# chengstone/cchess-zero

Hardware: AMD Instinct MI355X
Metric: MCTS simulations/sec (whole node), playout=1600, 7-block net (higher is better)
Workload: dtype mx6

## Files before the change

### cchess_zero_amd/csrc/cz_conv.hip

```cpp
#include "cz_internal.h"
#include "cz_conv_kernel.h"
#include "cz_trunk_split.h"
#include "cz_trunk_mx.h"
#ifdef CZ_EXPERIMENT_MX2
#include "cz_trunk_mx2.h"
#include <cstdlib>
#endif
#ifdef CZ_EXPERIMENT_MX12
#include "cz_trunk_mx12.h"
#include <cstdlib>
#endif

extern "C" int cz_conv3x3_c128_bf16(cz_ctx *c, const void *in, const void *wpk, const float *bias, const void *residual,
                                    void *out, int B, int relu) {
    using namespace czconv;
    CZ_REQUIRE(c && in && wpk && bias && out && B >= 0, "cz_conv3x3_c128_bf16: null argument");
    if (B == 0) return CZ_OK;
    if (!c->conv_attr_set) {
        CZ_HIP(hipFuncSetAttribute(reinterpret_cast<const void *>(k_conv3x3_c128), hipFuncAttributeMaxDynamicSharedMemorySize, CV_LDS_BYTES));
        c->conv_attr_set = true;
    }
    const int grid = (B + CV_P - 1) / CV_P;
    hipLaunchKernelGGL(k_conv3x3_c128, dim3(grid), dim3(CV_THREADS), CV_LDS_BYTES, c->stream, (const uint16_t *)in,
                       (const uint16_t *)wpk, bias, (const uint16_t *)residual, (uint16_t *)out, B, relu);
    CZ_HIP(hipGetLastError());
    return CZ_OK;
}

static unsigned long long *clock_probe(cz_ctx *c, int grid) {
    if (!c->clock_probe || grid > c->clock_probe_wgs) return nullptr;
    c->clock_probe_last_grid = grid;
    return c->clock_probe;
}

static int launch_tower(cz_ctx *c, const void *in, const void *wpk, const float *bias, void *out, const float *head_w,
                        const float *head_b, float *head_out, int B, int nblocks, const void *planes = nullptr,
                        const void *w0 = nullptr, const float *b0 = nullptr, bool f16 = false) {
    if (head_w && (reinterpret_cast<uintptr_t>(head_w) & 15u)) { cz_set_error("cz_net_trunk: head_w must be 16-byte aligned"); return CZ_EINVAL; }
    using namespace czconv;
    if (B == 0) return CZ_OK;
    if (!c->tower_attr_set) {
        CZ_HIP(hipFuncSetAttribute(reinterpret_cast<const void *>(k_tower8_c128<false, 4>), hipFuncAttributeMaxDynamicSharedMemorySize, T8_LDS_BYTES));
        CZ_HIP(hipFuncSetAttribute(reinterpret_cast<const void *>(k_tower8_c128<true, 4>), hipFuncAttributeMaxDynamicSharedMemorySize, T8_LDS_BYTES));
        c->tower_attr_set = true;
    }
    const int grid = (B + T8_P - 1) / T8_P;
    if (f16)
        hipLaunchKernelGGL((k_tower8_c128<true, 4>), dim3(grid), dim3(T8_THREADS), T8_LDS_BYTES, c->stream, (const uint16_t *)in,
                           (const uint16_t *)wpk, bias, (uint16_t *)out, head_w, head_b, head_out, (const uint16_t *)planes,
                           (const uint16_t *)w0, b0, B, 2 * nblocks, c->batch_count, clock_probe(c, grid));
    else
        hipLaunchKernelGGL((k_tower8_c128<false, 4>), dim3(grid), dim3(T8_THREADS), T8_LDS_BYTES, c->stream, (const uint16_t *)in,
                           (const uint16_t *)wpk, bias, (uint16_t *)out, head_w, head_b, head_out, (const uint16_t *)planes,
                           (const uint16_t *)w0, b0, B, 2 * nblocks, c->batch_count, clock_probe(c, grid));
    CZ_HIP(hipGetLastError());
    return CZ_OK;
}

extern "C" int cz_tower_c128_bf16(cz_ctx *c, const void *in, const void *wpk, const float *bias, void *out, int B, int nblocks) {
    CZ_REQUIRE(c && in && wpk && bias && out && B >= 0 && nblocks >= 1, "cz_tower_c128_bf16: null argument / nblocks < 1");
    return launch_tower(c, in, wpk, bias, out, nullptr, nullptr, nullptr, B, nblocks);
}

extern "C" int cz_tower_heads_c128_bf16(cz_ctx *c, const void *in, const void *wpk, const float *bias, void *trunk_out,
                                        const float *head_w, const float *head_b, float *head_out, int B, int nblocks) {
    CZ_REQUIRE(c && in && wpk && bias && head_w && head_b && head_out && B >= 0 && nblocks >= 1,
               "cz_tower_heads_c128_bf16: null argument / nblocks < 1");
    return launch_tower(c, in, wpk, bias, trunk_out, head_w, head_b, head_out, B, nblocks);
}

extern "C" int cz_net_trunk_bf16(cz_ctx *c, const void *planes16, const void *w0, const float *b0, const void *wpk,
                                 const float *bias, void *trunk_out, const float *head_w, const float *head_b,
                                 float *head_out, int B, int nblocks) {
    CZ_REQUIRE(c && planes16 && w0 && b0 && wpk && bias && B >= 0 && nblocks >= 1 && (trunk_out || head_out),
               "cz_net_trunk_bf16: null argument / nblocks < 1");
    CZ_REQUIRE(!head_out || (head_w && head_b), "cz_net_trunk_bf16: head_out needs head_w and head_b");
    return launch_tower(c, nullptr, wpk, bias, trunk_out, head_w, head_b, head_out, B, nblocks, planes16, w0, b0);
}

extern "C" int cz_net_trunk_f16(cz_ctx *c, const void *planes16, const void *w0, const float *b0, const void *wpk,
                                const float *bias, void *trunk_out, const float *head_w, const float *head_b,
                                float *head_out, int B, int nblocks) {
    CZ_REQUIRE(c && planes16 && w0 && b0 && wpk && bias && B >= 0 && nblocks >= 1 && (trunk_out || head_out),
               "cz_net_trunk_f16: null argument / nblocks < 1");
    CZ_REQUIRE(!head_out || (head_w && head_b), "cz_net_trunk_f16: head_out needs head_w and head_b");
    return launch_tower(c, nullptr, wpk, bias, trunk_out, head_w, head_b, head_out, B, nblocks, planes16, w0, b0, true);
}

extern "C" int cz_net_trunk_split(cz_ctx *c, const void *planes16, const void *w0, const float *b0, const void *wpk,
                                  const float *bias, float *trunk_out, const float *head_w, const float *head_b,
                                  float *head_out, int B, int nblocks, int halves_dtype) {
    using namespace czconv;
    CZ_REQUIRE(c && planes16 && w0 && b0 && wpk && bias && B >= 0 && nblocks >= 1 && (trunk_out || head_out),
               "cz_net_trunk_split: null argument / nblocks < 1");
    CZ_REQUIRE(!head_out || (head_w && head_b), "cz_net_trunk_split: head_out needs head_w and head_b");
    CZ_REQUIRE(halves_dtype == CZ_F16 || halves_dtype == CZ_BF16, "cz_net_trunk_split: halves_dtype must be CZ_F16 or CZ_BF16");
    if (head_w && (reinterpret_cast<uintptr_t>(head_w) & 15u)) { cz_set_error("cz_net_trunk_split: head_w must be 16-byte aligned"); return CZ_EINVAL; }
    if (B == 0) return CZ_OK;
    if (!c->split_attr_set) {
        CZ_HIP(hipFuncSetAttribute(reinterpret_cast<const void *>(k_trunk_split_c128<false>), hipFuncAttributeMaxDynamicSharedMemorySize, XS_LDS_BYTES));
        CZ_HIP(hipFuncSetAttribute(reinterpret_cast<const void *>(k_trunk_split_c128<true>), hipFuncAttributeMaxDynamicSharedMemorySize, XS_LDS_BYTES));
        c->split_attr_set = true;
    }
    const int grid = (B + XS_P - 1) / XS_P;
    if (halves_dtype == CZ_F16)
        hipLaunchKernelGGL((k_trunk_split_c128<true>), dim3(grid), dim3(XS_THREADS), XS_LDS_BYTES, c->stream, (const uint16_t *)wpk, bias,
                           trunk_out, head_w, head_b, head_out, (const uint16_t *)planes16, (const uint16_t *)w0, b0, B, 2 * nblocks,
                           c->batch_count, clock_probe(c, grid));
    else
        hipLaunchKernelGGL((k_trunk_split_c128<false>), dim3(grid), dim3(XS_THREADS), XS_LDS_BYTES, c->stream, (const uint16_t *)wpk, bias,
                           trunk_out, head_w, head_b, head_out, (const uint16_t *)planes16, (const uint16_t *)w0, b0, B, 2 * nblocks,
                           c->batch_count, clock_probe(c, grid));
    CZ_HIP(hipGetLastError());
    return CZ_OK;
}

extern "C" int cz_net_trunk_mx(cz_ctx *c, const void *planes16, const void *w0, const float *b0, const void *wpk, const float *bias,
                               float *trunk_out, const float *head_w, const float *head_b, float *head_out, int B, int nblocks) {
    using namespace czconv;
    CZ_REQUIRE(c && planes16 && w0 && b0 && wpk && bias && B >= 0 && nblocks >= 1 && (trunk_out || head_out),
               "cz_net_trunk_mx: null argument / nblocks < 1");
    CZ_REQUIRE(!head_out || (head_w && head_b), "cz_net_trunk_mx: head_out needs head_w and head_b");
    if (head_w && (reinterpret_cast<uintptr_t>(head_w) & 15u)) { cz_set_error("cz_net_trunk_mx: head_w must be 16-byte aligned"); return CZ_EINVAL; }
    if (reinterpret_cast<uintptr_t>(wpk) & 15u) { cz_set_error("cz_net_trunk_mx: wpk must be 16-byte aligned"); return CZ_EINVAL; }
    if (B == 0) return CZ_OK;
    const int grid = (B + MX_P - 1) / MX_P;
#ifdef CZ_EXPERIMENT_MX12
    {
        const char *e = getenv("CCHESS_MX_KERNEL");
        if (e && e[0] == '1' && e[1] == '2') {
            if (!c->mx2_attr_set) {
                CZ_HIP(hipFuncSetAttribute(reinterpret_cast<const void *>(k_trunk_mx12_c128), hipFuncAttributeMaxDynamicSharedMemorySize, MX_LDS_BYTES));
                c->mx2_attr_set = true;
            }
            hipLaunchKernelGGL(k_trunk_mx12_c128, dim3(grid), dim3(768), MX_LDS_BYTES, c->stream, (const unsigned char *)wpk, bias, trunk_out,
                               head_w, head_b, head_out, (const uint16_t *)planes16, (const uint16_t *)w0, b0, B, 2 * nblocks, c->batch_count,
                               clock_probe(c, grid));
            CZ_HIP(hipGetLastError());
            return CZ_OK;
        }
    }
#endif
#ifdef CZ_EXPERIMENT_MX2
    if (!c->mx_kernel) {
        const char *e = getenv("CCHESS_MX_KERNEL");
        c->mx_kernel = (e && e[0] == '2') ? 2 : 1;
    }
    if (c->mx_kernel == 2) {
        if (!c->mx2_attr_set) {
            CZ_HIP(hipFuncSetAttribute(reinterpret_cast<const void *>(k_trunk_mx2_c128), hipFuncAttributeMaxDynamicSharedMemorySize, MX_LDS_BYTES));
            c->mx2_attr_set = true;
        }
        const size_t need = (size_t)grid * MX2_XBUF_FLOATS_PER_WG * sizeof(float);
        if (need > c->mx_xbuf_bytes) {
            CZ_HIP(hipStreamSynchronize(c->stream));
            if (c->mx_xbuf) (void)hipFree(c->mx_xbuf);
            c->mx_xbuf = nullptr; c->mx_xbuf_bytes = 0;
            if (hipMalloc(&c->mx_xbuf, need) != hipSuccess) { c->mx_xbuf = nullptr; cz_set_error("cz_net_trunk_mx: hipMalloc(%zu B) for the block-input scratch failed", need); return CZ_ENOMEM; }
            c->mx_xbuf_bytes = need;
        }
        hipLaunchKernelGGL(k_trunk_mx2_c128, dim3(grid), dim3(MX_THREADS), MX_LDS_BYTES, c->stream, (const unsigned char *)wpk, bias, trunk_out,
                           head_w, head_b, head_out, (const uint16_t *)planes16, (const uint16_t *)w0, b0, B, 2 * nblocks, c->batch_count,
                           clock_probe(c, grid), (float *)c->mx_xbuf);
        CZ_HIP(hipGetLastError());
        return CZ_OK;
    }
#endif
    if (!c->mx_attr_set) {
        CZ_HIP(hipFuncSetAttribute(reinterpret_cast<const void *>(k_trunk_mx_c128), hipFuncAttributeMaxDynamicSharedMemorySize, MX_LDS_BYTES));
        c->mx_attr_set = true;
    }
    hipLaunchKernelGGL(k_trunk_mx_c128, dim3(grid), dim3(MX_THREADS), MX_LDS_BYTES, c->stream, (const unsigned char *)wpk, bias, trunk_out,
                       head_w, head_b, head_out, (const uint16_t *)planes16, (const uint16_t *)w0, b0, B, 2 * nblocks, c->batch_count,
                       clock_probe(c, grid));
    CZ_HIP(hipGetLastError());
    return CZ_OK;
}

extern "C" int cz_set_clock_probe(cz_ctx *c, unsigned long long *buf_dev, int max_workgroups) {
    CZ_REQUIRE(c && max_workgroups >= 0, "cz_set_clock_probe: null context");
    c->clock_probe = buf_dev;
    c->clock_probe_wgs = buf_dev ? max_workgroups : 0;
    c->clock_probe_last_grid = 0;
    return CZ_OK;
}

extern "C" int cz_clock_probe_last_grid(cz_ctx *c) { return c ? c->clock_probe_last_grid : 0; }
```

### cchess_zero_amd/csrc/cz_internal.h

```cpp
#pragma once
#include <cstddef>
#include <hip/hip_runtime.h>
#include <math.h>
#include <stdint.h>
#include <stdio.h>
#include <string>

#include "../../include/cchess_hip.h"
#include "cz_device.h"

void cz_set_error(const char *fmt, ...);
#define CZ_HIP(expr)                                                                              \
    do {                                                                                          \
        hipError_t _e = (expr);                                                                   \
        if (_e != hipSuccess) {                                                                   \
            cz_set_error("%s failed: %s (%s:%d)", #expr, hipGetErrorString(_e), __FILE__, __LINE__); \
            return CZ_EHIP;                                                                       \
        }                                                                                         \
    } while (0)
#define CZ_REQUIRE(cond, msg)                                \
    do {                                                     \
        if (!(cond)) { cz_set_error("%s", msg); return CZ_EINVAL; } \
    } while (0)

struct CzHostTables {
    char labels[CZ_NLABELS * 5];
    int16_t lut[CZ_NSQ * CZ_NSQ];
    int16_t unflip[CZ_NLABELS];
    uint16_t srcdst[CZ_NLABELS];
    uint64_t zob[15 * CZ_NSQ + 1];
};
const CzHostTables &cz_host_tables();

#define CZ_PATH_MAX 32

struct CzPool {
    float *P, *W, *Q;
    int32_t *N, *parent, *child_begin;
    uint16_t *child_count, *move;
    uint16_t *sd;
};

struct CzSelfplay {
    int max_plies;
    uint8_t *hist;
    int32_t *ply;
    uint8_t *stalled;
    uint8_t *active;
    uint8_t *start_board;
    uint8_t *start_side;
    int32_t *start_rr;
    long long *stats;
};

#define CZ_EC_BUCKETS 128
#define CZ_XC_BUSY (1ull << 63)
#define CZ_EC_ENTRIES (CZ_EC_BUCKETS * 64)
#ifndef CZ_EC_BUDGET
#define CZ_EC_BUDGET 4
#endif

struct CzTreeRec {
    int32_t root_rr, root_node, n_nodes, status;
    int32_t sims;
    int16_t last_depth;
    uint16_t root_ply;
    int32_t pend_kind, pend_leaf;
    float pend_value;
    int32_t pend_depth;
    uint32_t ec_hits, ec_lookups;
    unsigned long long pend_key;
    uint16_t pend_nmoves;
    uint8_t root_side, pend_side;
    uint32_t ec_collisions;
};
static_assert(sizeof(CzTreeRec) == 64, "CzTreeRec is one 64-byte line per tree");

template <typename T, int OFF>
struct CzRecField {
    char *base;
    __host__ __device__ __forceinline__ T &operator[](int g) const { return *reinterpret_cast<T *>(base + (size_t)g * sizeof(CzTreeRec) + OFF); }
};
#define CZ_REC_FIELD(type, name) CzRecField<type, offsetof(CzTreeRec, name)> name

struct CzTrees {
    CzPool pool;
    int cap;
    int words;
    unsigned long long *mark_bits;
    uint32_t *mark_rank;
    int32_t *adv_list, *adv_cnt;
    uint8_t *root_board;
    union {
        CzTreeRec *rec;
        CZ_REC_FIELD(int32_t, root_rr); CZ_REC_FIELD(int32_t, root_node); CZ_REC_FIELD(int32_t, n_nodes);
        CZ_REC_FIELD(int32_t, status); CZ_REC_FIELD(int32_t, sims); CZ_REC_FIELD(int16_t, last_depth); CZ_REC_FIELD(uint16_t, root_ply);
        CZ_REC_FIELD(int32_t, pend_kind); CZ_REC_FIELD(int32_t, pend_leaf); CZ_REC_FIELD(float, pend_value);
        CZ_REC_FIELD(int32_t, pend_depth); CZ_REC_FIELD(uint32_t, ec_hits); CZ_REC_FIELD(uint32_t, ec_lookups); CZ_REC_FIELD(uint32_t, ec_collisions);
        CZ_REC_FIELD(unsigned long long, pend_key); CZ_REC_FIELD(uint16_t, pend_nmoves);
        CZ_REC_FIELD(uint8_t, root_side); CZ_REC_FIELD(uint8_t, pend_side);
    };
    uint16_t *pend_moves;
    int32_t *pend_path;
    int32_t *pk_kind, *pk_leaf;
    float *pk_value;
    uint8_t *pk_side;
    uint16_t *pk_nmoves;
    unsigned long long *ec_key;
    int32_t *ec_node;
    float *ec_val;
    uint32_t *ec_board;
    uint32_t *pend_board;
    unsigned long long ec_key_mask;
    char *xc_base;
    uint32_t xc_mask;
    int32_t *slot_of;
    int32_t *evcnt;
    unsigned long long *evtotal;
};

struct cz_ctx {
    int device;
    hipStream_t stream;
    int max_games, cap, G;
    CzTables tab;
    void *tab_block;
    CzTrees t;
    void *tree_block;
    void *pool_block;
    bool adv_attr_set;
    bool adv_force_global;
    bool conv_attr_set, tower_attr_set, split_attr_set, mx_attr_set;
#if defined(CZ_EXPERIMENT_MX2) || defined(CZ_EXPERIMENT_MX12)
    bool mx2_attr_set;
    int mx_kernel;
    void *mx_xbuf;
    size_t mx_xbuf_bytes;
#endif
    int width;
    void *pend_block;
    int terminal_extra;
    int sim_target;
    int step_parity;
    const int32_t *batch_count;
    void *xc_block;
    int xc_log2_entries;
    const struct CzmTables *mask_tab;
    unsigned long long *clock_probe;
    int clock_probe_wgs, clock_probe_last_grid;
    CzSelfplay sp;
    void *sp_block;
    void *ec_block;
};

__host__ __device__ __forceinline__ size_t czx_n(const CzTrees &t) { return ((size_t)t.xc_mask + 1) * 64; }
__host__ __device__ __forceinline__ unsigned long long *czx_key(const CzTrees &t) { return reinterpret_cast<unsigned long long *>(t.xc_base); }
__host__ __device__ __forceinline__ uint32_t *czx_tree_stats(const CzTrees &t) { return reinterpret_cast<uint32_t *>(t.xc_base + czx_n(t) * 1088 + 64); }
__host__ __device__ __forceinline__ float *czx_val(const CzTrees &t) { return reinterpret_cast<float *>(t.xc_base + czx_n(t) * 8 + 64); }
__host__ __device__ __forceinline__ uint32_t *czx_cnt(const CzTrees &t) { return reinterpret_cast<uint32_t *>(t.xc_base + czx_n(t) * 12 + 64); }
__host__ __device__ __forceinline__ uint32_t *czx_board(const CzTrees &t) { return reinterpret_cast<uint32_t *>(t.xc_base + czx_n(t) * 16 + 64); }
__host__ __device__ __forceinline__ uint16_t *czx_moves(const CzTrees &t) { return reinterpret_cast<uint16_t *>(t.xc_base + czx_n(t) * 64 + 64); }
__host__ __device__ __forceinline__ uint16_t *czx_sd(const CzTrees &t) { return reinterpret_cast<uint16_t *>(t.xc_base + czx_n(t) * 320 + 64); }
__host__ __device__ __forceinline__ float *czx_P(const CzTrees &t) { return reinterpret_cast<float *>(t.xc_base + czx_n(t) * 576 + 64); }

struct TreeView {
    float *P, *W, *Q;
    int32_t *N, *parent, *child_begin;
    uint16_t *child_count, *move;
    uint16_t *sd;
};

__device__ __forceinline__ TreeView view_of(const CzTrees &t, int g) {
    const CzPool &p = t.pool;
    const size_t base = (size_t)g * (size_t)t.cap;
    TreeView v;
    v.P = p.P + base; v.W = p.W + base; v.Q = p.Q + base;
    v.N = p.N + base; v.parent = p.parent + base; v.child_begin = p.child_begin + base;
    v.child_count = p.child_count + base; v.move = p.move + base; v.sd = p.sd + base;
    return v;
}

__device__ __forceinline__ void init_root(TreeView v, int idx) {
    v.P[idx] = 1.0f;
    v.W[idx] = 0.f; v.Q[idx] = 0.f; v.N[idx] = 0; v.parent[idx] = -1; v.child_begin[idx] = -1;
    v.child_count[idx] = 0; v.move[idx] = 0xFFFF; v.sd[idx] = 0;
}

__device__ __forceinline__ void ec_clear_tree(const CzTrees &t, int g, int tid, int nthreads) {
    if (!t.ec_key) return;
    unsigned long long *k = t.ec_key + (size_t)g * CZ_EC_ENTRIES;
    for (int i = tid; i < CZ_EC_ENTRIES; i += nthreads) k[i] = 0ull;
}

__device__ __forceinline__ void fresh_root(const CzTrees &t, int g, int lane) {
    if (lane == 0) {
        t.root_node[g] = 0; t.n_nodes[g] = 1; t.status[g] = 0; t.sims[g] = 0; t.last_depth[g] = 0; t.root_ply[g] = 0;
        t.pend_kind[g] = 0; t.pend_leaf[g] = 0; t.pend_value[g] = 0.f; t.pend_side[g] = 0; t.pend_nmoves[g] = 0;
        init_root(view_of(t, g), 0);
    }
    ec_clear_tree(t, g, lane, 64);
}
__device__ __forceinline__ void fresh_root(const CzTrees &t, int g, int lane, const uint8_t *__restrict__ boards, int stride,
                                           const uint8_t *__restrict__ side, const int32_t *__restrict__ rr, int i) {
    for (int j = lane; j < CZD_BOARD_LDS; j += 64)
        t.root_board[(size_t)g * CZD_BOARD_LDS + j] = j < CZ_NSQ ? boards[(size_t)i * stride + j] : (uint8_t)0;
    if (lane == 0) { t.root_side[g] = side[i] ? 1 : 0; t.root_rr[g] = rr ? rr[i] : 0; }
    fresh_root(t, g, lane);
}

__device__ __forceinline__ void wave_kings_missing(const uint8_t *board, int lane, bool &Kmiss, bool &kmiss) {
    const int c0 = board[lane], c1 = (lane + 64 < CZ_NSQ) ? board[lane + 64] : 0;
    Kmiss = __ballot(c0 == 1 || c1 == 1) == 0ull;
    kmiss = __ballot(c0 == 8 || c1 == 8) == 0ull;
}
__device__ __forceinline__ int king_capture_winner(bool Kmiss) { return Kmiss ? 1 : 0; }
__device__ __forceinline__ bool restrict_round_draw(int rr) { return rr >= 60; }

__device__ __forceinline__ void root_children(const CzTrees &t, int g, const TreeView &v, int &cb, int &n) {
    const int root = t.root_node[g];
    cb = v.child_begin[root];
    n = cb < 0 ? 0 : (int)v.child_count[root];
}
__device__ __forceinline__ bool root_cannot_move(int status, int n) {
    return n == 0 || (status & (CZ_ST_NO_MOVES | CZ_ST_MOVE_OVERFLOW)) != 0;
}

__device__ __forceinline__ int wave_most_visited(const TreeView &v, int cb, int n, int lane) {
    int bn = -1, bi = 0x7fffffff;
    for (int i = lane; i < n; i += 64) {
        const int x = v.N[cb + i];
        if (x > bn) { bn = x; bi = i; }
    }
#pragma unroll
    for (int d = 32; d >= 1; d >>= 1) {
        const int on = __shfl_xor(bn, d, 64), oi = __shfl_xor(bi, d, 64);
        if (on > bn || (on == bn && oi < bi)) { bn = on; bi = oi; }
    }
    return bi;
}

__device__ __forceinline__ double wave_sum(double x) {
#pragma unroll
    for (int d = 32; d >= 1; d >>= 1) x += __shfl_xor(x, d, 64);
    return x;
}
__device__ __forceinline__ double wave_max(double x) {
#pragma unroll
    for (int d = 32; d >= 1; d >>= 1) x = fmax(x, __shfl_xor(x, d, 64));
    return x;
}
__device__ __forceinline__ double wave_incl_scan(double v, int lane) {
    double x = v;
#pragma unroll
    for (int d = 1; d < 64; d <<= 1) {
        const double y = __shfl_up(x, d, 64);
        if (lane >= d) x += y;
    }
    return x;
}

__device__ __forceinline__ void wave_visit_policy(const int N[2], int n, double inv_temp, int lane, double pi[2]) {
    double x[2], e[2];
#pragma unroll
    for (int r = 0; r < 2; ++r) {
        const int i = lane + 64 * r;
        x[r] = (i < n && N[r] > 0) ? inv_temp * log((double)N[r]) : -INFINITY;
    }
    const double m = wave_max(fmax(x[0], x[1]));
#pragma unroll
    for (int r = 0; r < 2; ++r) e[r] = (x[r] == -INFINITY || m == -INFINITY) ? 0.0 : exp(x[r] - m);
    const double se = wave_sum(e[0] + e[1]);
#pragma unroll
    for (int r = 0; r < 2; ++r) {
        const int i = lane + 64 * r;
        pi[r] = se > 0.0 ? e[r] / se : (i < n ? 1.0 / (double)n : 0.0);
    }
}

__device__ __forceinline__ int wave_pick_inverse_cdf(const double p[2], double u, int lane) {
    const double c0 = wave_incl_scan(p[0], lane);
    const double t0 = __shfl(c0, 63, 64);
    const double c1 = t0 + wave_incl_scan(p[1], lane);
    const double total = __shfl(c1, 63, 64);
    const double target = u * total;
    const unsigned long long h0 = __ballot(p[0] > 0.0 && c0 > target), h1 = __ballot(p[1] > 0.0 && c1 > target);
// ... 31 lines not shown
```

### cchess_zero_amd/csrc/cz_trunk_mx.h

```cpp
#pragma once
#include "cz_conv_kernel.h"

namespace czconv {

#include "cz_trunk_mx_asm.inc"

struct MXGeo {
    static constexpr int P = 2;
    static constexpr int ROWS = P * 90;
    static constexpr int THREADS = 512;
    static constexpr int ENT = 224;
    static constexpr int XPLANE = ENT * 16, YPLANE = ENT * 8, SPLANE = ENT * 4;
    static constexpr int X_OFF = 0, Y_OFF = 8 * XPLANE, S_OFF = Y_OFF + 8 * YPLANE;
    static constexpr int HI_OFF = S_OFF + 2 * SPLANE;
    static constexpr int ZERO_OFF = HI_OFF + ROWS * CV_ROWB;
    static constexpr int W_OFF = ZERO_OFF + CV_ROWB;
    static constexpr int SLAB_BYTES = 16384;
    static constexpr int SLAB_SHIFT = 14;
    static constexpr int SLABS_PER_LAYER = 36;
    static constexpr int LDS_BYTES = W_OFF + TW_NBUF * SLAB_BYTES;
    static constexpr int PLANES_OFF = W_OFF + 3 * SLAB_BYTES;
    static constexpr int HEADW_OFF = LDS_BYTES;
    static constexpr int LDS_TOTAL = LDS_BYTES + 3 * 128 * 4;
    static constexpr int F32_ROWB = 512;
};
static_assert(MXGeo::HI_OFF % 256 == 0 && MXGeo::W_OFF % 16 == 0, "hi rows are swizzled by their absolute 256-byte row");
static_assert(MXGeo::Y_OFF == 28672 && MXGeo::S_OFF == 43008, "tools/gen_tower_asm.py: MX_Y_OFF / MX_S_OFF");
static_assert(MXGeo::ROWS * MXGeo::F32_ROWB <= MXGeo::HEADW_OFF, "fp32 trunk rows must leave the head weights alone");
constexpr int MX_P = MXGeo::P, MX_THREADS = MXGeo::THREADS, MX_LDS_BYTES = MXGeo::LDS_TOTAL;

typedef unsigned u32x6 __attribute__((ext_vector_type(6)));
typedef _Float16 f16x8 __attribute__((ext_vector_type(8)));

__device__ __forceinline__ u32x6 mx_cvt6(f32x16 a, f32x16 b, float scale) {
    u32x6 r;
    asm volatile("v_cvt_scalef32_2xpk16_fp6_f32 %0, %1, %2, %3" : "=&v"(r) : "v"(a), "v"(b), "v"(scale));
    return r;
}

__global__ __launch_bounds__(512, 2) void k_trunk_mx_c128(const unsigned char *__restrict__ wpk,
                                                           const float *__restrict__ bias,
                                                           float *__restrict__ out,
                                                           const float *__restrict__ head_w,
                                                           const float *__restrict__ head_b,
                                                           float *__restrict__ head_out,
                                                           const uint16_t *__restrict__ planes,
                                                           const uint16_t *__restrict__ w0,
                                                           const float *__restrict__ b0,
                                                           int B, int nlayers,
                                                           const int *__restrict__ bcount,
                                                           unsigned long long *__restrict__ clk) {
    extern __shared__ __attribute__((aligned(16))) unsigned char smem[];
    using Geo = MXGeo;
    const int tid = threadIdx.x, lane = tid & 63, wave = tid >> 6;
    const int wr = wave >> 2, ct = wave & 3;
    const int l31 = lane & 31, khalf = lane >> 5;
    const int pos0 = blockIdx.x * Geo::P;
    if (bcount) {
        const int live = *bcount;
        B = live < B ? live : B;
    }
    if (pos0 >= B) return;
    unsigned long long clk_c0 = 0, clk_r0 = 0;
    if (clk) { clk_c0 = __builtin_readcyclecounter(); clk_r0 = __builtin_amdgcn_s_memrealtime(); }
    const int npos = (B - pos0) < Geo::P ? (B - pos0) : Geo::P;
    const int nrows = npos * 90;
    const int nslabs = nlayers * Geo::SLABS_PER_LAYER;
    auto lds_addr = [](int row_byte_off, int c) { return row_byte_off + ((c ^ ((row_byte_off >> 8) & 15)) << 4); };
    const unsigned voff0 = (unsigned)tid << 4, voff1 = voff0 + (unsigned)Geo::THREADS * 16u;
    const int wave_u = __builtin_amdgcn_readfirstlane(wave);
    auto lds_row_of = [](int natural) {
        const int p = natural / 90, c = natural - p * 90, y = c / 10, x = c - y * 10;
        return 20 * y + 10 * p + x;
    };

    auto dma_slab = [&](int slab) {
        const unsigned char *src = wpk + (size_t)slab * Geo::SLAB_BYTES;
        unsigned char *dst = smem + Geo::W_OFF + ((unsigned)slab & 3u) * Geo::SLAB_BYTES + (wave_u << 10);
        __builtin_amdgcn_global_load_lds((const __attribute__((address_space(1))) void *)(src + voff0),
                                         (__attribute__((address_space(3))) void *)dst, 16, 0, 0);
        __builtin_amdgcn_global_load_lds((const __attribute__((address_space(1))) void *)(src + voff1),
                                         (__attribute__((address_space(3))) void *)(dst + Geo::THREADS * 16), 16, 0, 0);
    };
    for (int q = 0; q < 3; ++q) dma_slab(q < nslabs ? q : nslabs - 1);
    {
        const uint4 *g = reinterpret_cast<const uint4 *>(planes + (size_t)pos0 * 90 * 16);
        for (int idx = tid; idx < Geo::ROWS * 2; idx += Geo::THREADS) {
            uint4 v = make_uint4(0, 0, 0, 0);
            if (idx < nrows * 2) v = g[idx];
            *reinterpret_cast<uint4 *>(smem + Geo::PLANES_OFF + (idx << 4)) = v;
        }
    }
    if (tid < 16) *reinterpret_cast<uint4 *>(smem + Geo::ZERO_OFF + (tid << 4)) = make_uint4(0, 0, 0, 0);
    if (tid < 256) *reinterpret_cast<uint4 *>(smem + Geo::X_OFF + (tid >> 5) * Geo::XPLANE + (192 + (tid & 31)) * 16) = make_uint4(0, 0, 0, 0);
    else *reinterpret_cast<uint2 *>(smem + Geo::Y_OFF + ((tid - 256) >> 5) * Geo::YPLANE + (192 + (tid & 31)) * 8) = make_uint2(0, 0);
    if (tid < 64) *reinterpret_cast<uint32_t *>(smem + Geo::S_OFF + (tid >> 5) * Geo::SPLANE + (192 + (tid & 31)) * 4) = 0x7f7f7f7fu;
    if (head_out && tid < 3 * 128 / 4)
        reinterpret_cast<float4 *>(smem + Geo::HEADW_OFF)[tid] = reinterpret_cast<const float4 *>(head_w)[tid];
    bf16x8 wf[9][2];
#pragma unroll
    for (int t = 0; t < 9; ++t)
#pragma unroll
        for (int part = 0; part < 2; ++part)
            wf[t][part] = *reinterpret_cast<const bf16x8 *>(w0 + ((size_t)(((t * 2 + part) * 2 + khalf) * 128 + ct * 32 + l31) << 3));
    asm volatile("s_waitcnt vmcnt(0)" ::: "memory");
    __syncthreads();

    int rowk[3], tapmask[3], natb[3];
#pragma unroll
    for (int i = 0; i < 3; ++i) {
        const int k = 32 * (wr * 3 + i) + l31 - 12;
        const int kk = k < 0 ? 0 : k;
        const int h = kk / 20, rem = kk - h * 20, pp = rem / 10, w = rem - pp * 10;
        rowk[i] = k;
        natb[i] = (pp * 90 + h * 10 + w) * 32;
        int m = 0;
        for (int t = 0; t < 9; ++t) {
            const int y = h + t / 3 - 1, x = w + t % 3 - 1;
            if (k >= 0 && y >= 0 && y < 9 && x >= 0 && x < 10) m |= 1 << t;
        }
        tapmask[i] = m;
    }
    auto tap_addr = [&](int tap, int (&ab)[3], int (&key)[3], int (&xr)[3], int (&yr)[3]) {
        const int delta = (tap / 3 - 1) * 20 + (tap - (tap / 3) * 3 - 1);
#pragma unroll
        for (int i = 0; i < 3; ++i) {
            const int kk = rowk[i] + delta;
            const bool on = (tapmask[i] >> tap) & 1;
            const int rb = Geo::HI_OFF + kk * CV_ROWB;
            ab[i] = on ? rb : Geo::ZERO_OFF;
            key[i] = ((rb >> 8) & 15) ^ khalf;
            xr[i] = khalf * Geo::XPLANE + ((on ? kk : 192 + (kk & 31)) << 4);
            yr[i] = xr[i] >> 1;
        }
    };
    const int vb0 = Geo::W_OFF + khalf * 2048 + ((ct * 32 + l31) << 4);
    const int vy0 = Geo::W_OFF + 12288 + khalf * 1024 + ((ct * 32 + l31) << 3);
    const int vs0 = Geo::W_OFF + 14336 + khalf * 512 + ((ct * 32 + l31) << 2);
    int keep;

    int rkk[3];
    auto refresh_rk = [&]() {
#pragma unroll
        for (int i = 0; i < 3; ++i) {
            rkk[i] = rowk[i] < 0 ? 0 : rowk[i];
            asm volatile("" : "+v"(rkk[i]));
        }
    };
    f32x16 xreg[3];
    float4 bqn[4];
    auto load_bias = [&](const float *bl) {
        int t = threadIdx.x;
        asm volatile("" : "+v"(t));
        const int boff = ((t >> 6) & 3) * 32 + 4 * ((t & 63) >> 5);
#pragma unroll
        for (int q = 0; q < 4; ++q) bqn[q] = *reinterpret_cast<const float4 *>(bl + boff + 8 * q);
    };
    auto init_acc = [&](f32x16 (&acc)[3], const float *bl, bool add_x) {
#pragma unroll
        for (int q = 0; q < 4; ++q) {
            const float4 bq = bl ? *reinterpret_cast<const float4 *>(bl + ct * 32 + 8 * q + 4 * khalf) : bqn[q];
#pragma unroll
            for (int i = 0; i < 3; ++i) {
                acc[i][4 * q + 0] = bq.x + (add_x ? xreg[i][4 * q + 0] : 0.0f);
                acc[i][4 * q + 1] = bq.y + (add_x ? xreg[i][4 * q + 1] : 0.0f);
                acc[i][4 * q + 2] = bq.z + (add_x ? xreg[i][4 * q + 2] : 0.0f);
                acc[i][4 * q + 3] = bq.w + (add_x ? xreg[i][4 * q + 3] : 0.0f);
            }
        }
    };
    auto store_tile = [&](f32x16 a, int i, bool keep_x) {
        f32x16 v;
#pragma unroll
        for (int r = 0; r < 16; ++r) v[r] = __builtin_amdgcn_fmed3f(a[r], 0.0f, 65504.0f);
        if (keep_x) xreg[i] = v;
        uint32_t pk[8];
        f32x16 hi, lo;
#pragma unroll
        for (int r = 0; r < 16; r += 2) {
            pk[r >> 1] = pack_pair<true>(f32x2{v[r], v[r + 1]});
            const f32x2 u = unpack_pair<true>(pk[r >> 1]);
            hi[r] = u[0]; hi[r + 1] = u[1];
            lo[r] = (v[r] - u[0]) * 2048.0f; lo[r + 1] = (v[r + 1] - u[1]) * 2048.0f;
        }
        float m = v[0];
#pragma unroll
        for (int r = 1; r < 16; ++r) m = fmaxf(m, v[r]);
        int byte = (int)(__float_as_uint(m) >> 23) - 2;
        byte = byte < 1 ? 1 : byte;
        const u32x6 blk = mx_cvt6(hi, lo, __uint_as_float((uint32_t)byte << 23));
        const bool live = rowk[i] >= 0;
        if (live) {
            const int rowb = Geo::HI_OFF + rkk[i] * CV_ROWB;
#pragma unroll
            for (int q = 0; q < 4; ++q) {
                const int n0 = ct * 32 + 8 * q + 4 * khalf;
                *reinterpret_cast<uint2 *>(smem + lds_addr(rowb, n0 >> 3) + ((n0 & 4) << 1)) = make_uint2(pk[2 * q], pk[2 * q + 1]);
            }
            const int g = 2 * ct + khalf;
            *reinterpret_cast<uint4 *>(smem + Geo::X_OFF + g * Geo::XPLANE + (rkk[i] << 4)) = make_uint4(blk[0], blk[1], blk[2], blk[3]);
            *reinterpret_cast<uint2 *>(smem + Geo::Y_OFF + g * Geo::YPLANE + (rkk[i] << 3)) = make_uint2(blk[4], blk[5]);
            smem[Geo::S_OFF + khalf * Geo::SPLANE + (rkk[i] << 2) + ct] = (unsigned char)byte;
        }
    };
    auto store_tile_f32 = [&](f32x16 a, int i) {
        if (rowk[i] < 0) return;
#pragma unroll
        for (int q = 0; q < 4; ++q) {
            const int c = 8 * ct + 2 * q + khalf;
            *reinterpret_cast<float4 *>(smem + rkk[i] * Geo::F32_ROWB + ((c ^ (rkk[i] & 31)) << 4)) =
                make_float4(fmaxf(a[4 * q + 0], 0.0f), fmaxf(a[4 * q + 1], 0.0f), fmaxf(a[4 * q + 2], 0.0f), fmaxf(a[4 * q + 3], 0.0f));
        }
    };

    {
        f32x16 acc[3];
        init_acc(acc, b0, false);
        load_bias(bias);
#pragma unroll
        for (int t = 0; t < 9; ++t) {
            const int shift = (t / 3 - 1) * 10 + (t % 3 - 1);
            bf16x8 af[3];
#pragma unroll
            for (int i = 0; i < 3; ++i) {
                const int a = ((tapmask[i] >> t) & 1) ? Geo::PLANES_OFF + (natb[i] + shift * 32) : Geo::ZERO_OFF;
                af[i] = *reinterpret_cast<const bf16x8 *>(smem + a + khalf * 16);
            }
#pragma unroll
            for (int part = 0; part < 2; ++part)
#pragma unroll
                for (int i = 0; i < 3; ++i)
                    acc[i] = mfma_32x32x16<true>(wf[t][part], af[i], acc[i]);
        }
        refresh_rk();
#pragma unroll
        for (int i = 0; i < 3; ++i) store_tile(acc[i], i, true);
        __syncthreads();
    }

#define MX_OPERANDS(NAB, NKEY)                                                                                       \
            : [c0] "+v"(acc[0]), [c1] "+v"(acc[1]), [c2] "+v"(acc[2]),                                                 \
              [a0h0] "+v"(fa.a[0]), [a0h1] "+v"(fa.a[1]), [a0h2] "+v"(fa.a[2]), [w0] "+v"(fa.w),                      \
              [a1h0] "+v"(fb.a[0]), [a1h1] "+v"(fb.a[1]), [a1h2] "+v"(fb.a[2]), [w1] "+v"(fb.w),                      \
              [sb0] "+v"(sb[0]), [sb1] "+v"(sb[1]), [sb2] "+v"(sb[2]),                                                \
              [t0] "=&v"(t0), [t1] "=&v"(t1), [t2] "=&v"(t2), [ws] "=&v"(wsr), [keep] "=&s"(keep)                      \
            : [ab0] "v"(ab[0]), [ab1] "v"(ab[1]), [ab2] "v"(ab[2]), [key0] "v"(key[0]), [key1] "v"(key[1]),            \
              [key2] "v"(key[2]), [nab0] "v"(NAB[0]), [nab1] "v"(NAB[1]), [nab2] "v"(NAB[2]), [nkey0] "v"(NKEY[0]),     \
              [nkey1] "v"(NKEY[1]), [nkey2] "v"(NKEY[2]), [xr0] "v"(xr[0]), [xr1] "v"(xr[1]), [xr2] "v"(xr[2]),        \
              [yr0] "v"(yr[0]), [yr1] "v"(yr[1]), [yr2] "v"(yr[2]), [vb] "v"(vb), [vy] "v"(vy), [vs] "v"(vs),          \
              [vbn] "v"(vbn), [voff0] "v"(voff0), [voff1] "v"(voff1), [sbase] "s"(sbase), [ldst] "s"(ldst)
#define MX_CLOBBERS "memory", "scc", "v232", "v233", "v234", "v235", "v236", "v237", "v238", "v239", "v240", "v241", "v242", "v243", \
                    "v244", "v245", "v246", "v247", "v248", "v249", "v250", "v251", "v252", "v253", "v254", "v255"
#define MX_ARGS()                                                                                                    \
            const int slot = ((unsigned)g & 3u) << Geo::SLAB_SHIFT;                                                  \
            const int vb = vb0 + slot, vy = vy0 + slot, vs = vs0 + slot;                                             \
            const int vbn = vb0 + ((((unsigned)g + 1u) & 3u) << Geo::SLAB_SHIFT);                                    \
            const int gn = g + 3 < nslabs ? g + 3 : nslabs - 1;                                                      \
            const unsigned char *sbase = wpk + (size_t)gn * Geo::SLAB_BYTES;                                         \
            const int ldst = Geo::W_OFF + ((((unsigned)g + 3u) & 3u) << Geo::SLAB_SHIFT) + (wave_u << 10);
#define MX_RUN(ASMSTR, NAB, NKEY)                                                                                    \
        {                                                                                                            \
            MX_ARGS()                                                                                                \
            asm volatile(ASMSTR MX_OPERANDS(NAB, NKEY) : MX_CLOBBERS);                                               \
            ++g;                                                                                                     \
        }
#define MX_RUNV(ASMSTR, NAB, NKEY)                           \
        {                                                                                                            \
            MX_ARGS()                                                                                                \
            asm volatile(ASMSTR MX_OPERANDS(NAB, NKEY), [skipm] "s"(skipm) : MX_CLOBBERS, "vcc");                    \
            ++g;                                                                                                     \
        }

#ifdef MX_TIMING
    unsigned long long tm_loop = 0, tm_epi = 0, tm_set = 0, tm_t0 = __builtin_readcyclecounter();
    const unsigned long long tm_first = tm_t0 - clk_c0;
#define MX_TM(acc) { const unsigned long long n_ = __builtin_readcyclecounter(); acc += n_ - tm_t0; tm_t0 = n_; }
#else
#define MX_TM(acc)
#endif
    struct MxFrag { bf16x8 a[3], w; };
    int g = 0;
    int skipm;
    asm volatile("s_cmp_lt_u32 %1, 4\n\ts_cselect_b32 %0, 1, 0" : "=s"(skipm) : "s"(wave_u) : "scc");
#pragma unroll 1
    for (int layer = 0; layer < nlayers; ++layer) {
        f32x16 acc[3];
        init_acc(acc, nullptr, (layer & 1) != 0);
        int ab[3], key[3], nab[3], nkey[3], xr[3], yr[3], nxr[3], nyr[3], t0, t1, t2, wsr;
        int sb[3] = {0, 0, 0};
        MxFrag fa, fb;
        tap_addr(0, ab, key, xr, yr);
        {
            const int vb = vb0 + (((unsigned)g & 3u) << Geo::SLAB_SHIFT);
#pragma unroll
            for (int i = 0; i < 3; ++i) {
                fa.a[i] = *reinterpret_cast<const bf16x8 *>(smem + ab[i] + ((0 ^ key[i]) << 4));
                fb.a[i] = *reinterpret_cast<const bf16x8 *>(smem + ab[i] + ((2 ^ key[i]) << 4));
            }
            fa.w = *reinterpret_cast<const bf16x8 *>(smem + vb);
            fb.w = *reinterpret_cast<const bf16x8 *>(smem + vb + 4096);
            asm volatile("" : "+v"(fa.a[0]), "+v"(fa.a[1]), "+v"(fa.a[2]), "+v"(fa.w), "+v"(fb.a[0]), "+v"(fb.a[1]), "+v"(fb.a[2]), "+v"(fb.w));
        }
        MX_TM(tm_set)
        int tap = 0;
#pragma unroll 1
        for (; tap < 3; ++tap) {
            MX_RUNV(MX_SKIP0_ASM_Q0, ab, key)
            MX_RUNV(MX_SKIP0_ASM_Q1, ab, key)
            MX_RUNV(MX_SKIP0_ASM_Q2, ab, key)
            tap_addr(tap + 1, nab, nkey, nxr, nyr);
            MX_RUNV(MX_SKIP0_ASM_Q3, nab, nkey)
#pragma unroll
            for (int i = 0; i < 3; ++i) { ab[i] = nab[i]; key[i] = nkey[i]; xr[i] = nxr[i]; yr[i] = nyr[i]; }
        }
#pragma unroll 1
        for (; tap < 8; ++tap) {
            MX_RUN(MX_SLAB_ASM_Q0, ab, key)
            MX_RUN(MX_SLAB_ASM_Q1, ab, key)
            MX_RUN(MX_SLAB_ASM_Q2, ab, key)
            tap_addr(tap + 1, nab, nkey, nxr, nyr);
            MX_RUN(MX_SLAB_ASM_Q3, nab, nkey)
#pragma unroll
            for (int i = 0; i < 3; ++i) { ab[i] = nab[i]; key[i] = nkey[i]; xr[i] = nxr[i]; yr[i] = nyr[i]; }
        }
        MX_RUN(MX_SLAB_ASM_Q0, ab, key)
        MX_RUN(MX_SLAB_ASM_Q1, ab, key)
        MX_RUN(MX_SLAB_ASM_Q2, ab, key)
        MX_RUN(MX_SLAB_ASM_Q3_LAST, ab, key)
        const bool last = layer + 1 == nlayers;
        if (last) asm volatile("s_waitcnt vmcnt(0)" ::: "memory");
        else load_bias(bias + (layer + 1) * 128);
        asm volatile("s_nop 15\n\ts_nop 15\n\ts_nop 15" ::: "memory");
        MX_TM(tm_loop)
        refresh_rk();
        if (last) {
#pragma unroll
            for (int i = 0; i < 3; ++i) store_tile_f32(acc[i], i);
        } else {
#pragma unroll
            for (int i = 0; i < 3; ++i) store_tile(acc[i], i, (layer & 1) != 0);
        }
        __syncthreads();
        MX_TM(tm_epi)
    }
    if (clk && tid == 0) {
        clk[blockIdx.x * 4 + 0] = clk_c0; clk[blockIdx.x * 4 + 1] = __builtin_readcyclecounter();
        clk[blockIdx.x * 4 + 2] = clk_r0; clk[blockIdx.x * 4 + 3] = __builtin_amdgcn_s_memrealtime();
#ifdef MX_TIMING
        clk[blockIdx.x * 4 + 0] = tm_first; clk[blockIdx.x * 4 + 1] = tm_loop; clk[blockIdx.x * 4 + 2] = tm_epi; clk[blockIdx.x * 4 + 3] = tm_set;
#endif
    }
    asm volatile("s_waitcnt vmcnt(0)" ::: "memory");
    if (out) {
        float4 *go = reinterpret_cast<float4 *>(out + (size_t)pos0 * 90 * 128);
        for (int idx = tid; idx < nrows * 32; idx += Geo::THREADS) {
            const int r = idx >> 5, c = idx & 31, k = lds_row_of(r);
            go[idx] = *reinterpret_cast<const float4 *>(smem + k * Geo::F32_ROWB + ((c ^ (k & 31)) << 4));
        }
    }
    if (head_out) {
        const float *hw = reinterpret_cast<const float *>(smem + Geo::HEADW_OFF);
        for (int r = tid; r < nrows; r += Geo::THREADS) {
            const int k = lds_row_of(r);
            float acc0 = 0.f, acc1 = 0.f, acc2 = 0.f;
#pragma unroll 4
            for (int c = 0; c < 32; ++c) {
                const float4 e = *reinterpret_cast<const float4 *>(smem + k * Geo::F32_ROWB + ((c ^ (k & 31)) << 4));
                const float *w0_ = hw + c * 4, *w1_ = hw + 128 + c * 4, *w2_ = hw + 256 + c * 4;
                acc0 += e.x * w0_[0] + e.y * w0_[1] + e.z * w0_[2] + e.w * w0_[3];
                acc1 += e.x * w1_[0] + e.y * w1_[1] + e.z * w1_[2] + e.w * w1_[3];
                acc2 += e.x * w2_[0] + e.y * w2_[1] + e.z * w2_[2] + e.w * w2_[3];
            }
            float *o = head_out + ((size_t)pos0 * 90 + r) * 3;
            o[0] = fmaxf(acc0 + head_b[0], 0.f);
            o[1] = fmaxf(acc1 + head_b[1], 0.f);
            o[2] = fmaxf(acc2 + head_b[2], 0.f);
        }
    }
}
#undef MX_OPERANDS
#undef MX_CLOBBERS
#undef MX_ARGS
#undef MX_RUN
#undef MX_RUNV

}
```

Measured before the change: 2.000 million.

## Make MX trunk kernel persistent over position pairs with cross-pair weight prefetch

Caps the MX trunk launch at one workgroup per CU and loops each workgroup over position pairs. The slab DMA ring wraps into the next pair's first slabs, and the next pair's planes, first-layer weights and bias are requested before the current pair's epilogue. This hides the per-workgroup startup and weight-prefetch latency. The fp32 output rows move under the ring and behind the input planes so buffers 0..2 stay free for prefetch, and the head projection is spread across threads one channel each. The cost is serialising pairs within a CU, which leaves only one workgroup resident per CU even though launch bounds allow two, and more complex LDS aliasing.

```diff
diff --git a/cchess_zero_amd/csrc/cz_conv.hip b/cchess_zero_amd/csrc/cz_conv.hip
--- a/cchess_zero_amd/csrc/cz_conv.hip
+++ b/cchess_zero_amd/csrc/cz_conv.hip
@@ -168,11 +168,14 @@
 #endif
     if (!c->mx_attr_set) {
         CZ_HIP(hipFuncSetAttribute(reinterpret_cast<const void *>(k_trunk_mx_c128), hipFuncAttributeMaxDynamicSharedMemorySize, MX_LDS_BYTES));
+        hipDeviceProp_t prop;
+        CZ_HIP(hipGetDeviceProperties(&prop, c->device));
+        c->mx_cus = prop.multiProcessorCount > 0 ? prop.multiProcessorCount : 1;
         c->mx_attr_set = true;
     }
-    hipLaunchKernelGGL(k_trunk_mx_c128, dim3(grid), dim3(MX_THREADS), MX_LDS_BYTES, c->stream, (const unsigned char *)wpk, bias, trunk_out,
-                       head_w, head_b, head_out, (const uint16_t *)planes16, (const uint16_t *)w0, b0, B, 2 * nblocks, c->batch_count,
-                       clock_probe(c, grid));
+    hipLaunchKernelGGL(k_trunk_mx_c128, dim3(grid < c->mx_cus ? grid : c->mx_cus), dim3(MX_THREADS), MX_LDS_BYTES, c->stream,
+                       (const unsigned char *)wpk, bias, trunk_out, head_w, head_b, head_out, (const uint16_t *)planes16,
+                       (const uint16_t *)w0, b0, B, 2 * nblocks, c->batch_count, clock_probe(c, grid));
     CZ_HIP(hipGetLastError());
     return CZ_OK;
 }
diff --git a/cchess_zero_amd/csrc/cz_internal.h b/cchess_zero_amd/csrc/cz_internal.h
--- a/cchess_zero_amd/csrc/cz_internal.h
+++ b/cchess_zero_amd/csrc/cz_internal.h
@@ -131,6 +131,7 @@
     bool adv_attr_set;
     bool adv_force_global;
     bool conv_attr_set, tower_attr_set, split_attr_set, mx_attr_set;
+    int mx_cus;
 #if defined(CZ_EXPERIMENT_MX2) || defined(CZ_EXPERIMENT_MX12)
     bool mx2_attr_set;
     int mx_kernel;
diff --git a/cchess_zero_amd/csrc/cz_trunk_mx.h b/cchess_zero_amd/csrc/cz_trunk_mx.h
--- a/cchess_zero_amd/csrc/cz_trunk_mx.h
+++ b/cchess_zero_amd/csrc/cz_trunk_mx.h
@@ -23,10 +23,15 @@
     static constexpr int HEADW_OFF = LDS_BYTES;
     static constexpr int LDS_TOTAL = LDS_BYTES + 3 * 128 * 4;
     static constexpr int F32_ROWB = 512;
+    static constexpr int F32_LOW_ROWS = W_OFF / F32_ROWB;
+    static constexpr int F32_HIGH_OFF = PLANES_OFF + 8192;
 };
 static_assert(MXGeo::HI_OFF % 256 == 0 && MXGeo::W_OFF % 16 == 0, "hi rows are swizzled by their absolute 256-byte row");
 static_assert(MXGeo::Y_OFF == 28672 && MXGeo::S_OFF == 43008, "tools/gen_tower_asm.py: MX_Y_OFF / MX_S_OFF");
-static_assert(MXGeo::ROWS * MXGeo::F32_ROWB <= MXGeo::HEADW_OFF, "fp32 trunk rows must leave the head weights alone");
+static_assert(MXGeo::W_OFF % MXGeo::F32_ROWB == 0 && MXGeo::ROWS * 32 <= 8192 &&
+              MXGeo::F32_HIGH_OFF + (MXGeo::ROWS - MXGeo::F32_LOW_ROWS) * MXGeo::F32_ROWB <= MXGeo::LDS_BYTES,
+              "fp32 trunk rows: under the ring, then in buffer 3 behind the input planes; never in buffers 0..2 or the head weights");
+static_assert(MXGeo::SLABS_PER_LAYER % TW_NBUF == 0, "a pair's slab g and the next pair's slab g share a ring buffer");
 constexpr int MX_P = MXGeo::P, MX_THREADS = MXGeo::THREADS, MX_LDS_BYTES = MXGeo::LDS_TOTAL;
 
 typedef unsigned u32x6 __attribute__((ext_vector_type(6)));
@@ -55,16 +60,15 @@
     const int tid = threadIdx.x, lane = tid & 63, wave = tid >> 6;
     const int wr = wave >> 2, ct = wave & 3;
     const int l31 = lane & 31, khalf = lane >> 5;
-    const int pos0 = blockIdx.x * Geo::P;
     if (bcount) {
         const int live = *bcount;
         B = live < B ? live : B;
     }
-    if (pos0 >= B) return;
+    const int npairs = (B + Geo::P - 1) / Geo::P;
+    int pair = blockIdx.x;
+    if (pair >= npairs) return;
     unsigned long long clk_c0 = 0, clk_r0 = 0;
     if (clk) { clk_c0 = __builtin_readcyclecounter(); clk_r0 = __builtin_amdgcn_s_memrealtime(); }
-    const int npos = (B - pos0) < Geo::P ? (B - pos0) : Geo::P;
-    const int nrows = npos * 90;
     const int nslabs = nlayers * Geo::SLABS_PER_LAYER;
     auto lds_addr = [](int row_byte_off, int c) { return row_byte_off + ((c ^ ((row_byte_off >> 8) & 15)) << 4); };
     const unsigned voff0 = (unsigned)tid << 4, voff1 = voff0 + (unsigned)Geo::THREADS * 16u;
@@ -83,37 +87,50 @@
                                          (__attribute__((address_space(3))) void *)(dst + Geo::THREADS * 16), 16, 0, 0);
     };
     for (int q = 0; q < 3; ++q) dma_slab(q < nslabs ? q : nslabs - 1);
-    {
-        const uint4 *g = reinterpret_cast<const uint4 *>(planes + (size_t)pos0 * 90 * 16);
-        for (int idx = tid; idx < Geo::ROWS * 2; idx += Geo::THREADS) {
-            uint4 v = make_uint4(0, 0, 0, 0);
-            if (idx < nrows * 2) v = g[idx];
-            *reinterpret_cast<uint4 *>(smem + Geo::PLANES_OFF + (idx << 4)) = v;
-        }
-    }
-    if (tid < 16) *reinterpret_cast<uint4 *>(smem + Geo::ZERO_OFF + (tid << 4)) = make_uint4(0, 0, 0, 0);
-    if (tid < 256) *reinterpret_cast<uint4 *>(smem + Geo::X_OFF + (tid >> 5) * Geo::XPLANE + (192 + (tid & 31)) * 16) = make_uint4(0, 0, 0, 0);
-    else *reinterpret_cast<uint2 *>(smem + Geo::Y_OFF + ((tid - 256) >> 5) * Geo::YPLANE + (192 + (tid & 31)) * 8) = make_uint2(0, 0);
-    if (tid < 64) *reinterpret_cast<uint32_t *>(smem + Geo::S_OFF + (tid >> 5) * Geo::SPLANE + (192 + (tid & 31)) * 4) = 0x7f7f7f7fu;
     if (head_out && tid < 3 * 128 / 4)
         reinterpret_cast<float4 *>(smem + Geo::HEADW_OFF)[tid] = reinterpret_cast<const float4 *>(head_w)[tid];
+    uint4 pv;
     bf16x8 wf[9][2];
-#pragma unroll
-    for (int t = 0; t < 9; ++t)
-#pragma unroll
-        for (int part = 0; part < 2; ++part)
-            wf[t][part] = *reinterpret_cast<const bf16x8 *>(w0 + ((size_t)(((t * 2 + part) * 2 + khalf) * 128 + ct * 32 + l31) << 3));
+    float4 bqn[4];
+    auto load_bias = [&](const float *bl) {
+        int t = threadIdx.x;
+        asm volatile("" : "+v"(t));
+        const int boff = ((t >> 6) & 3) * 32 + 4 * ((t & 63) >> 5);
+#pragma unroll
+        for (int q = 0; q < 4; ++q) bqn[q] = *reinterpret_cast<const float4 *>(bl + boff + 8 * q);
+    };
+    auto wide = [](int lo) {
+        unsigned hi = 0;
+        asm volatile("" : "+v"(hi));
+        return (size_t)(((unsigned long long)hi << 32) | (unsigned)lo);
+    };
+    auto request_pair = [&](int p) {
+        const int live2 = ((B - p * Geo::P) < Geo::P ? (B - p * Geo::P) : Geo::P) * 90 * 2;
+        int ti = threadIdx.x;
+        asm volatile("" : "+v"(ti));
+        { unsigned z = 0; asm volatile("" : "+v"(z)); pv = make_uint4(z, z, z, z); }
+        if (ti < live2) pv = reinterpret_cast<const uint4 *>(planes + (size_t)p * Geo::P * 90 * 16)[wide(ti)];
+        const int wfo = (((ti >> 5) & 1) * 128 + ((ti >> 6) & 3) * 32 + (ti & 31)) << 3;
+        const uint16_t *w0p = w0;
+        const float *b0p = b0;
+        asm volatile("" : "+s"(w0p), "+s"(b0p));
+#pragma unroll
+        for (int t = 0; t < 9; ++t)
+#pragma unroll
+            for (int part = 0; part < 2; ++part)
+                wf[t][part] = *reinterpret_cast<const bf16x8 *>(w0p + wide(wfo) + (t * 2 + part) * 2 * 128 * 8);
+        load_bias(b0p);
+    };
+    request_pair(pair);
     asm volatile("s_waitcnt vmcnt(0)" ::: "memory");
-    __syncthreads();
-
-    int rowk[3], tapmask[3], natb[3];
+
+    int rowk[3], tapmask[3];
 #pragma unroll
     for (int i = 0; i < 3; ++i) {
         const int k = 32 * (wr * 3 + i) + l31 - 12;
         const int kk = k < 0 ? 0 : k;
         const int h = kk / 20, rem = kk - h * 20, pp = rem / 10, w = rem - pp * 10;
         rowk[i] = k;
-        natb[i] = (pp * 90 + h * 10 + w) * 32;
         int m = 0;
         for (int t = 0; t < 9; ++t) {
             const int y = h + t / 3 - 1, x = w + t % 3 - 1;
@@ -137,7 +154,6 @@
     const int vb0 = Geo::W_OFF + khalf * 2048 + ((ct * 32 + l31) << 4);
     const int vy0 = Geo::W_OFF + 12288 + khalf * 1024 + ((ct * 32 + l31) << 3);
     const int vs0 = Geo::W_OFF + 14336 + khalf * 512 + ((ct * 32 + l31) << 2);
-    int keep;
 
     int rkk[3];
     auto refresh_rk = [&]() {
@@ -148,18 +164,10 @@
         }
     };
     f32x16 xreg[3];
-    float4 bqn[4];
-    auto load_bias = [&](const float *bl) {
-        int t = threadIdx.x;
-        asm volatile("" : "+v"(t));
-        const int boff = ((t >> 6) & 3) * 32 + 4 * ((t & 63) >> 5);
-#pragma unroll
-        for (int q = 0; q < 4; ++q) bqn[q] = *reinterpret_cast<const float4 *>(bl + boff + 8 * q);
-    };
-    auto init_acc = [&](f32x16 (&acc)[3], const float *bl, bool add_x) {
+    auto init_acc = [&](f32x16 (&acc)[3], bool add_x) {
 #pragma unroll
         for (int q = 0; q < 4; ++q) {
-            const float4 bq = bl ? *reinterpret_cast<const float4 *>(bl + ct * 32 + 8 * q + 4 * khalf) : bqn[q];
+            const float4 bq = bqn[q];
 #pragma unroll
             for (int i = 0; i < 3; ++i) {
                 acc[i][4 * q + 0] = bq.x + (add_x ? xreg[i][4 * q + 0] : 0.0f);
@@ -203,19 +211,56 @@
             smem[Geo::S_OFF + khalf * Geo::SPLANE + (rkk[i] << 2) + ct] = (unsigned char)byte;
         }
     };
+    auto f32_row = [](int k) {
+        return k < Geo::F32_LOW_ROWS ? k * Geo::F32_ROWB : Geo::F32_HIGH_OFF + (k - Geo::F32_LOW_ROWS) * Geo::F32_ROWB;
+    };
     auto store_tile_f32 = [&](f32x16 a, int i) {
         if (rowk[i] < 0) return;
 #pragma unroll
         for (int q = 0; q < 4; ++q) {
             const int c = 8 * ct + 2 * q + khalf;
-            *reinterpret_cast<float4 *>(smem + rkk[i] * Geo::F32_ROWB + ((c ^ (rkk[i] & 31)) << 4)) =
+            *reinterpret_cast<float4 *>(smem + f32_row(rkk[i]) + ((c ^ (rkk[i] & 31)) << 4)) =
                 make_float4(fmaxf(a[4 * q + 0], 0.0f), fmaxf(a[4 * q + 1], 0.0f), fmaxf(a[4 * q + 2], 0.0f), fmaxf(a[4 * q + 3], 0.0f));
         }
     };
 
+    int keep;
+    int skipm;
+    asm volatile("s_cmp_lt_u32 %1, 4\n\ts_cselect_b32 %0, 1, 0" : "=s"(skipm) : "s"(wave_u) : "scc");
+#pragma unroll 1
+    for (;;) {
+    const int pos0 = pair * Geo::P;
+    const int npos = (B - pos0) < Geo::P ? (B - pos0) : Geo::P;
+    const int nrows = npos * 90;
+    const int next = pair + (int)gridDim.x;
+    const bool more = next < npairs;
     {
+        int ti = threadIdx.x;
+        unsigned z = 0;
+        asm volatile("" : "+v"(ti), "+v"(z));
+        if (ti < Geo::ROWS * 2) *reinterpret_cast<uint4 *>(smem + Geo::PLANES_OFF + (ti << 4)) = pv;
+        if (ti < 16) *reinterpret_cast<uint4 *>(smem + Geo::ZERO_OFF + (ti << 4)) = make_uint4(z, z, z, z);
+        if (ti < 256) *reinterpret_cast<uint4 *>(smem + Geo::X_OFF + (ti >> 5) * Geo::XPLANE + (192 + (ti & 31)) * 16) = make_uint4(z, z, z, z);
+        else *reinterpret_cast<uint2 *>(smem + Geo::Y_OFF + ((ti - 256) >> 5) * Geo::YPLANE + (192 + (ti & 31)) * 8) = make_uint2(z, z);
+        if (ti < 64) *reinterpret_cast<uint32_t *>(smem + Geo::S_OFF + (ti >> 5) * Geo::SPLANE + (192 + (ti & 31)) * 4) = 0x7f7f7f7fu;
+    }
+    __syncthreads();
+
+    {
+        int natb[3], tmk[3];
+        int ti = threadIdx.x;
+        asm volatile("" : "+v"(ti));
+#pragma unroll
+        for (int i = 0; i < 3; ++i) {
+            const int k = 32 * ((ti >> 8) * 3 + i) + (ti & 31) - 12;
+            tmk[i] = tapmask[i];
+            asm volatile("" : "+v"(tmk[i]));
+            const int kk = k < 0 ? 0 : k;
+            const int h = kk / 20, rem = kk - h * 20, pp = rem / 10, w = rem - pp * 10;
+            natb[i] = (pp * 90 + h * 10 + w) * 32;
+        }
         f32x16 acc[3];
-        init_acc(acc, b0, false);
+        init_acc(acc, false);
         load_bias(bias);
 #pragma unroll
         for (int t = 0; t < 9; ++t) {
@@ -223,7 +268,7 @@
             bf16x8 af[3];
 #pragma unroll
             for (int i = 0; i < 3; ++i) {
-                const int a = ((tapmask[i] >> t) & 1) ? Geo::PLANES_OFF + (natb[i] + shift * 32) : Geo::ZERO_OFF;
+                const int a = ((tmk[i] >> t) & 1) ? Geo::PLANES_OFF + (natb[i] + shift * 32) : Geo::ZERO_OFF;
                 af[i] = *reinterpret_cast<const bf16x8 *>(smem + a + khalf * 16);
             }
 #pragma unroll
@@ -255,7 +300,7 @@
             const int slot = ((unsigned)g & 3u) << Geo::SLAB_SHIFT;                                                  \
             const int vb = vb0 + slot, vy = vy0 + slot, vs = vs0 + slot;                                             \
             const int vbn = vb0 + ((((unsigned)g + 1u) & 3u) << Geo::SLAB_SHIFT);                                    \
-            const int gn = g + 3 < nslabs ? g + 3 : nslabs - 1;                                                      \
+            const int gn = g + 3 < nslabs ? g + 3 : (more ? g + 3 - nslabs : nslabs - 1);    \
             const unsigned char *sbase = wpk + (size_t)gn * Geo::SLAB_BYTES;                                         \
             const int ldst = Geo::W_OFF + ((((unsigned)g + 3u) & 3u) << Geo::SLAB_SHIFT) + (wave_u << 10);
 #define MX_RUN(ASMSTR, NAB, NKEY)                                                                                    \
@@ -280,12 +325,10 @@
 #endif
     struct MxFrag { bf16x8 a[3], w; };
     int g = 0;
-    int skipm;
-    asm volatile("s_cmp_lt_u32 %1, 4\n\ts_cselect_b32 %0, 1, 0" : "=s"(skipm) : "s"(wave_u) : "scc");
 #pragma unroll 1
     for (int layer = 0; layer < nlayers; ++layer) {
         f32x16 acc[3];
-        init_acc(acc, nullptr, (layer & 1) != 0);
+        init_acc(acc, (layer & 1) != 0);
         int ab[3], key[3], nab[3], nkey[3], xr[3], yr[3], nxr[3], nyr[3], t0, t1, t2, wsr;
         int sb[3] = {0, 0, 0};
         MxFrag fa, fb;
@@ -328,8 +371,7 @@
         MX_RUN(MX_SLAB_ASM_Q2, ab, key)
         MX_RUN(MX_SLAB_ASM_Q3_LAST, ab, key)
         const bool last = layer + 1 == nlayers;
-        if (last) asm volatile("s_waitcnt vmcnt(0)" ::: "memory");
-        else load_bias(bias + (layer + 1) * 128);
+        if (!last) load_bias(bias + (layer + 1) * 128);
         asm volatile("s_nop 15\n\ts_nop 15\n\ts_nop 15" ::: "memory");
         MX_TM(tm_loop)
         refresh_rk();
@@ -343,39 +385,58 @@
         __syncthreads();
         MX_TM(tm_epi)
     }
-    if (clk && tid == 0) {
-        clk[blockIdx.x * 4 + 0] = clk_c0; clk[blockIdx.x * 4 + 1] = __builtin_readcyclecounter();
-        clk[blockIdx.x * 4 + 2] = clk_r0; clk[blockIdx.x * 4 + 3] = __builtin_amdgcn_s_memrealtime();
+    if (clk && threadIdx.x == 0) {
+        unsigned long long *ck = clk + (size_t)pair * 4 + wide(0);
+        ck[0] = clk_c0; ck[1] = __builtin_readcyclecounter();
+        ck[2] = clk_r0; ck[3] = __builtin_amdgcn_s_memrealtime();
 #ifdef MX_TIMING
-        clk[blockIdx.x * 4 + 0] = tm_first; clk[blockIdx.x * 4 + 1] = tm_loop; clk[blockIdx.x * 4 + 2] = tm_epi; clk[blockIdx.x * 4 + 3] = tm_set;
+        ck[0] = tm_first; ck[1] = tm_loop; ck[2] = tm_epi; ck[3] = tm_set;
 #endif
     }
-    asm volatile("s_waitcnt vmcnt(0)" ::: "memory");
+    if (clk) { clk_c0 = __builtin_readcyclecounter(); clk_r0 = __builtin_amdgcn_s_memrealtime(); }
+    request_pair(more ? next : pair);
+    int tt = threadIdx.x;
+    asm volatile("" : "+v"(tt));
     if (out) {
         float4 *go = reinterpret_cast<float4 *>(out + (size_t)pos0 * 90 * 128);
-        for (int idx = tid; idx < nrows * 32; idx += Geo::THREADS) {
+        for (int idx = tt; idx < nrows * 32; idx += Geo::THREADS) {
             const int r = idx >> 5, c = idx & 31, k = lds_row_of(r);
-            go[idx] = *reinterpret_cast<const float4 *>(smem + k * Geo::F32_ROWB + ((c ^ (k & 31)) << 4));
-        }
-    }
+            go[wide(idx)] = *reinterpret_cast<const float4 *>(smem + f32_row(k) + ((c ^ (k & 31)) << 4));
+        }
+    }
+    float hv[2] = {0.f, 0.f};
     if (head_out) {
         const float *hw = reinterpret_cast<const float *>(smem + Geo::HEADW_OFF);
-        for (int r = tid; r < nrows; r += Geo::THREADS) {
-            const int k = lds_row_of(r);
-            float acc0 = 0.f, acc1 = 0.f, acc2 = 0.f;
+#pragma unroll
+        for (int j = 0; j < 2; ++j) {
+            const int item = tt + j * Geo::THREADS;
+            if (item < 3 * nrows) {
+                const int ch = item / nrows, r = item - ch * nrows, k = lds_row_of(r);
+                const float *w_ = hw + ch * 128;
+                float a = 0.f;
 #pragma unroll 4
-            for (int c = 0; c < 32; ++c) {
-                const float4 e = *reinterpret_cast<const float4 *>(smem + k * Geo::F32_ROWB + ((c ^ (k & 31)) << 4));
-                const float *w0_ = hw + c * 4, *w1_ = hw + 128 + c * 4, *w2_ = hw + 256 + c * 4;
-                acc0 += e.x * w0_[0] + e.y * w0_[1] + e.z * w0_[2] + e.w * w0_[3];
-                acc1 += e.x * w1_[0] + e.y * w1_[1] + e.z * w1_[2] + e.w * w1_[3];
-                acc2 += e.x * w2_[0] + e.y * w2_[1] + e.z * w2_[2] + e.w * w2_[3];
-            }
-            float *o = head_out + ((size_t)pos0 * 90 + r) * 3;
-            o[0] = fmaxf(acc0 + head_b[0], 0.f);
-            o[1] = fmaxf(acc1 + head_b[1], 0.f);
-            o[2] = fmaxf(acc2 + head_b[2], 0.f);
-        }
+                for (int c = 0; c < 32; ++c) {
+                    const float4 e = *reinterpret_cast<const float4 *>(smem + f32_row(k) + ((c ^ (k & 31)) << 4));
+                    a += e.x * w_[c * 4 + 0] + e.y * w_[c * 4 + 1] + e.z * w_[c * 4 + 2] + e.w * w_[c * 4 + 3];
+                }
+                hv[j] = fmaxf(a + head_b[wide(ch)], 0.f);
+            }
+        }
+    }
+    asm volatile("s_waitcnt vmcnt(0)" ::: "memory");
+    if (head_out) {
+#pragma unroll
+        for (int j = 0; j < 2; ++j) {
+            const int item = tt + j * Geo::THREADS;
+            if (item < 3 * nrows) {
+                const int ch = item / nrows, r = item - ch * nrows;
+                (head_out + (size_t)pos0 * 90 * 3)[wide(r * 3 + ch)] = hv[j];
+            }
+        }
+    }
+    if (!more) break;
+    pair = next;
+    __syncthreads();
     }
 }
 #undef MX_OPERANDS
```

Measured after the change: 1.932 million, median of 2. -3.4%, worse.
